# valohai/distributed-llms-example

Hardware: AMD Instinct MI355X
Metric: samples/sec (whole node) T5-base summarization fine-tune at 1/2/4/8 MI355X (higher is better)
Workload: dtype bf16; 1 GPU; model=t5-base, global_batch=512, per_gpu_batch=512, grad_accum=1, seq_len=1024, target_len=128, parallelism=dp1, grad_ckpt=False, grad_dtype=float32, backend=none, world_size=1, comm_stress=False, hip_graph=True

## Files before the change

csrc/attn.hip:

```cpp
#include "common.h"
#include "route.h"
#include "attn_params.h"
#include "attn_tile.h"
#include <stdlib.h>
#include <type_traits>

using namespace dllm;

DLLM_SEED_STEP_TU(attn)

namespace {

static_assert(HG == RW_G, "attention Weyl step = the row-Weyl hash's");
DLLM_DEVICE uint32_t pair_y(uint32_t g) { return rw_pair_y(g); }
DLLM_DEVICE uint32_t pair_gbase(uint32_t rh, uint32_t kp0) { return rw_gbase(rh, kp0); }
DLLM_DEVICE uint32_t drop_mask2(uint32_t y, uint32_t t2) { return rw_drop2(y, t2); }

DLLM_DEVICE constexpr int keep_bit(int t, int i) { return ((i & 1) << 4) + 8 * t + (i >> 1); }
DLLM_DEVICE uint32_t pair_slot_kp(int p) { return (uint32_t)((p & 1) + 4 * ((p & 7) >> 1) + 16 * (p >> 3)); }

DLLM_DEVICE uint32_t dropout_word(uint32_t rh, int kbase, int hh, uint32_t thr) {
  const uint32_t gbase = pair_gbase(rh, (uint32_t)(kbase >> 1) + 2u * (uint32_t)hh);
  const uint32_t t2 = ((thr - 0x8000u) & 0xFFFFu) * 0x10001u;
  uint32_t drop = 0;
// ... 557 lines not shown
    for (int i = 0; i < 2; ++i) {
      const uint32_t qq = (uint32_t)min(qt * K2_QT + drow[i], P.Sq - 1);
      const uint32_t dst = base + (uint32_t)((2 * w + i) * 1024);
      bld16(qbase_p, __umul24(qq, qss2) + dc16[i], __builtin_amdgcn_readfirstlane(dst));
      bld16(dbase_p, __umul24(qq, dss2) + dc16[i], __builtin_amdgcn_readfirstlane(dst + TILE64 * 2));
    }
    glds4(rec_src + (long)qt * 256, __builtin_amdgcn_readfirstlane(base + 4 * TILE64 + w * 256));
    if (DROP) glds4(keep_src + qt * K2_QT, __builtin_amdgcn_readfirstlane(base + 4 * TILE64 + 1024 + w * 256));
  };
  constexpr int DPT = DROP ? 6 : 5;

  if (qt_begin < nqt_all) issue(0, qt_begin);
  if (NB == 3 && qt_begin + 1 < nqt_all) issue(1, qt_begin + 1);
  if (HAS_BIAS) {
    const float* lrow = P.lut + (long)h * L;
    for (int t = tid; t < win + K2_QT; t += 256) {
      const int i = win - 1 - t, gi = k0 + i;
      lut_r[t] = (i >= 0 && gi < L) ? lrow[gi] * LOG2E : 0.f;
    }
    for (int i = tid; i < win; i += 256) dlut_s[i] = 0.f;
  }
  float sat_acc_lo = 0.f, sat_acc_hi = 0.f;
  bool key_ok = false;
  if (tid < BWD_BK) {
    const int kk = k0 + tid;
    key_ok = kk < P.Sk;
    if (HAS_KPM && key_ok) key_ok = P.kpm[(long)b * P.Sk + kk] != 0;
    kmask[tid] = key_ok ? 0.f : -INFINITY;
  }
  const bool block_live = !HAS_KPM || __syncthreads_or(key_ok ? 1 : 0);
  const bool block_masked = __syncthreads_or((tid < BWD_BK && !key_ok) ? 1 : 0);
  bf16x8v kf[4], vf[4];
  {
    const uint16_t* kp = P.k + b * P.k_sb + (long)key * P.k_ss + h * P.k_sh;
    const uint16_t* vp = P.v + b * P.v_sb + (long)key * P.v_ss + h * P.v_sh;
#pragma unroll
    for (int s = 0; s < 4; ++s) {
      u16x8 a = {0, 0, 0, 0, 0, 0, 0, 0}, c = a;
      if (kvalid) {
        a = *reinterpret_cast<const u16x8*>(kp + 16 * s + 8 * hh);
        c = *reinterpret_cast<const u16x8*>(vp + 16 * s + 8 * hh);
      }
      kf[s] = as_frag(a);
      vf[s] = as_frag(c);
    }
  }
  asm volatile("" ::"v"(kf[0]), "v"(kf[1]), "v"(kf[2]), "v"(kf[3]), "v"(vf[0]), "v"(vf[1]), "v"(vf[2]), "v"(vf[3]));
  const float km = kmask[w * 32 + r];
  const int kl = key - k0, kc = kl & 31;
  const int mcol = (kl >> 6) * 2 + ((kc >> 2) & 1);
  const int mbit = keep_bit((kl >> 5) & 1, (kc & 3) + 4 * (kc >> 3));
  const float dscale = DROP ? 1.f / (1.f - P.p_drop) : 1.f;
  const uint32_t dsbits = __float_as_uint(dscale);

  const int nqt = block_live ? nqt_all : qt_begin;
  if (!block_live) wait_vm<0>();
  f32x16 dv0 = {}, dv1 = {}, dk0 = {}, dk1 = {};
  auto stage = [&](int qt, auto slot_c) __attribute__((always_inline)) {
    constexpr int SLOT = decltype(slot_c)::value;
    if (NB == 3 && qt + 1 < nqt) wait_vm<DPT>();
    else wait_vm<0>();
    __syncthreads();
    if (qt + NB - 1 < nqt) issue((SLOT + NB - 1) % NB, qt + NB - 1);
    const unsigned char* stg = smem + SLOT * K2_STAGE;
    const uint16_t* Qb = reinterpret_cast<const uint16_t*>(stg);
    const uint16_t* dOb = Qb + TILE64;
    const float* rec = reinterpret_cast<const float*>(stg + 4 * TILE64);
    const uint32_t* mwd = reinterpret_cast<const uint32_t*>(stg + 4 * TILE64 + 1024);
#pragma unroll
    for (int u = 0; u < 2; ++u) {
      const int q0 = qt * K2_QT + 32 * u;
      f32x16 sacc = {}, dpacc = {};
      if constexpr (NB == 3) {
        bf16x8v qa[4], da[4];
#pragma unroll
        for (int s = 0; s < 4; ++s) {
          qa[s] = as_frag(ld_row(Qb, 32 * u + r, 2 * s + hh));
          da[s] = as_frag(ld_row(dOb, 32 * u + r, 2 * s + hh));
        }
        __builtin_amdgcn_sched_barrier(0);
#pragma unroll
        for (int s = 0; s < 4; ++s) {
          sacc = mfma32(qa[s], kf[s], sacc);
          dpacc = mfma32(da[s], vf[s], dpacc);
        }
      } else {
#pragma unroll
        for (int s = 0; s < 4; ++s) {
          sacc = mfma32(as_frag(ld_row(Qb, 32 * u + r, 2 * s + hh)), kf[s], sacc);
          dpacc = mfma32(as_frag(ld_row(dOb, 32 * u + r, 2 * s + hh)), vf[s], dpacc);
        }
      }
      const int sat = !HAS_BIAS ? 0
                      : (kw0 + 31 - q0 + P.Sq - 1 <= P.sat_lo ? 1 : (kw0 - q0 - 31 + P.Sq - 1 >= P.sat_hi ? 2 : 0));
      const bool use_lut = HAS_BIAS && sat == 0;
      f32x16 pd, ds;
      if constexpr (NB == 3) {
        const float* rt_row = rec + (use_lut ? 0 : (sat == 1 ? 64 : 128)) + 32 * u + 4 * hh;
        const float* nd_row = rec + 192 + 32 * u + 4 * hh;
        float rt[16], nd[16];
        uint32_t mw[16];
#pragma unroll
        for (int g = 0; g < 4; ++g) {
          const f32x4 a = *reinterpret_cast<const f32x4*>(rt_row + 8 * g);
          const f32x4 c = *reinterpret_cast<const f32x4*>(nd_row + 8 * g);
#pragma unroll
          for (int e = 0; e < 4; ++e) {
            rt[4 * g + e] = a[e];
            nd[4 * g + e] = c[e];
          }
          if (DROP) {
            const u32x4 v = *reinterpret_cast<const u32x4*>(mwd + mcol * 64 + 32 * u + 8 * g + 4 * hh);
#pragma unroll
            for (int e = 0; e < 4; ++e) mw[4 * g + e] = v[e];
          }
        }
        if (use_lut) {
          const float* lrow_t = lut_r + (win - 1 - (key - q0 - 4 * hh + P.Sq - 1 - k0));
#pragma unroll
          for (int i0 = 0; i0 < 16; i0 += 8) {
            float lv[8];
#pragma unroll
            for (int i = 0; i < 8; ++i) lv[i] = lrow_t[crow(i0 + i, 0)];
#pragma unroll
            for (int i = 0; i < 8; ++i) rt[i0 + i] += lv[i];
          }
        }
        if (block_masked) {
#pragma unroll
          for (int i = 0; i < 16; ++i) rt[i] += km;
        }
        const bool tile_causal = CAUSAL && (kw0 + 31 > q0 + P.causal_off);
#pragma unroll
        for (int i = 0; i < 16; ++i) {
          const float x = fmaf(sacc[i], sl2, rt[i]);
          float pr = fast_exp2(x);
          if (CAUSAL && tile_causal && key > q0 + crow(i, hh) + P.causal_off) pr = 0.f;
          float keepf = 1.f;
          if (DROP) keepf = __uint_as_float((uint32_t)__builtin_amdgcn_sbfe((int)mw[i], mbit, 1) & dsbits);
          pd[i] = pr * keepf;
          ds[i] = pr * fmaf(dpacc[i], keepf, nd[i]);
        }
      } else {
        const float* rt_row = rec + (use_lut ? 0 : (sat == 1 ? 64 : 128)) + 32 * u + 4 * hh;
        const float* nd_row = rec + 192 + 32 * u + 4 * hh;
        const float* lrow_t = lut_r + (win - 1 - (key - q0 - 4 * hh + P.Sq - 1 - k0));
        const bool tile_causal = CAUSAL && (kw0 + 31 > q0 + P.causal_off);
#pragma unroll
        for (int g = 0; g < 4; ++g) {
          f32x4 rt4 = *reinterpret_cast<const f32x4*>(rt_row + 8 * g);
          const f32x4 nd4 = *reinterpret_cast<const f32x4*>(nd_row + 8 * g);
          u32x4 mw4 = {0u, 0u, 0u, 0u};
          if (DROP) mw4 = *reinterpret_cast<const u32x4*>(mwd + mcol * 64 + 32 * u + 8 * g + 4 * hh);
#pragma unroll
          for (int e = 0; e < 4; ++e) {
            const int i = 4 * g + e;
            float t = rt4[e];
            if (use_lut) t += lrow_t[crow(i, 0)];
            if (block_masked) t += km;
            float pr = fast_exp2(fmaf(sacc[i], sl2, t));
            if (CAUSAL && tile_causal && key > q0 + crow(i, hh) + P.causal_off) pr = 0.f;
            float keepf = 1.f;
            if (DROP) keepf = __uint_as_float((uint32_t)__builtin_amdgcn_sbfe((int)mw4[e], mbit, 1) & dsbits);
            sacc[i] = pr * keepf;
            dpacc[i] = pr * fmaf(dpacc[i], keepf, nd4[e]);
          }
        }
        pd = sacc;
        ds = dpacc;
      }
      if (HAS_BIAS && sat != 0) {
        float t = 0.f;
#pragma unroll
        for (int i = 0; i < 16; ++i) t += ds[i];
        if (sat == 1) sat_acc_lo += t;
        else sat_acc_hi += t;
      } else if (HAS_BIAS) {
        const int rb = r + 4 * hh;
        float tot = 0.f, neg = 0.f;
#pragma unroll
        for (int i0 = 0; i0 < 16; i0 += 8) {
          float v[8];
#pragma unroll
          for (int i = 0; i < 8; ++i) v[i] = __shfl(ds[i0 + i], ((rb + crow(i0 + i, 0)) & 31) + 32 * hh, 64);
#pragma unroll
          for (int i = 0; i < 8; ++i) {
            tot += v[i];
            neg += rb + crow(i0 + i, 0) < 32 ? 0.f : v[i];
          }
        }
        tot += __shfl_xor(tot, 32, 64);
        neg += __shfl_xor(neg, 32, 64);
        const int li = w * 32 + r - q0 + P.Sq - 1;
        const int la = hh == 0 ? li : li - 32;
        const float va = hh == 0 ? tot - neg : (li >= 32 ? neg : 0.f);
        atomicAdd(&dlut_s[la < 0 ? 0 : la], va);
      }
      const bf16x8v pf0 = pack8(pd, 0), pf1 = pack8(pd, 8), sf0 = pack8(ds, 0), sf1 = pack8(ds, 8);
      if constexpr (NB == 3) {
        bf16x8v ot[2][2], qtr[2][2];
#pragma unroll
        for (int sp = 0; sp < 2; ++sp) {
          const int c0 = 32 * u + 16 * sp + 4 * hh;
#pragma unroll
          for (int t = 0; t < 2; ++t) {
            ot[sp][t] = ld_tr_operand(dOb, c0, t, r);
            qtr[sp][t] = ld_tr_operand(Qb, c0, t, r);
          }
        }
        __builtin_amdgcn_sched_barrier(0);
#pragma unroll
        for (int sp = 0; sp < 2; ++sp) {
          const bf16x8v pfv = sp == 0 ? pf0 : pf1, sfv = sp == 0 ? sf0 : sf1;
          dv0 = mfma32(ot[sp][0], pfv, dv0);
          dv1 = mfma32(ot[sp][1], pfv, dv1);
          dk0 = mfma32(qtr[sp][0], sfv, dk0);
          dk1 = mfma32(qtr[sp][1], sfv, dk1);
        }
      } else {
#pragma unroll
        for (int sp = 0; sp < 2; ++sp) {
          const int c0 = 32 * u + 16 * sp + 4 * hh;
          const bf16x8v pfv = sp == 0 ? pf0 : pf1, sfv = sp == 0 ? sf0 : sf1;
          dv0 = mfma32(ld_tr_operand(dOb, c0, 0, r), pfv, dv0);
          dv1 = mfma32(ld_tr_operand(dOb, c0, 1, r), pfv, dv1);
          dk0 = mfma32(ld_tr_operand(Qb, c0, 0, r), sfv, dk0);
          dk1 = mfma32(ld_tr_operand(Qb, c0, 1, r), sfv, dk1);
        }
      }
    }
  };
  for (int qt = qt_begin; qt < nqt; qt += NB) {
    stage(qt, std::integral_constant<int, 0>{});
    if (qt + 1 < nqt) stage(qt + 1, std::integral_constant<int, 1>{});
    if constexpr (NB == 3) {
      if (qt + 2 < nqt) stage(qt + 2, std::integral_constant<int, 2>{});
    }
  }

  {
    __syncthreads();
    unsigned char* scr = smem + w * 8192;
#pragma unroll
    for (int t = 0; t < 2; ++t) {
      const f32x16& ak = t == 0 ? dk0 : dk1;
      const f32x16& av = t == 0 ? dv0 : dv1;
#pragma unroll
      for (int g = 0; g < 4; ++g) {
        u16x4 pk = {f2bf(ak[4 * g] * P.scale), f2bf(ak[4 * g + 1] * P.scale), f2bf(ak[4 * g + 2] * P.scale),
                    f2bf(ak[4 * g + 3] * P.scale)};
        u16x4 pv = {f2bf(av[4 * g]), f2bf(av[4 * g + 1]), f2bf(av[4 * g + 2]), f2bf(av[4 * g + 3])};
        const int off = r * 128 + (((4 * t + g) ^ (r & 7)) << 4) + 8 * hh;
        *reinterpret_cast<u16x4*>(scr + off) = pk;
        *reinterpret_cast<u16x4*>(scr + 4096 + off) = pv;
      }
    }
    asm volatile("s_waitcnt lgkmcnt(0)" ::: "memory");
    float ak[8] = {0.f, 0.f, 0.f, 0.f, 0.f, 0.f, 0.f, 0.f}, av[8] = {0.f, 0.f, 0.f, 0.f, 0.f, 0.f, 0.f, 0.f};
#pragma unroll
    for (int st = 0; st < 4; ++st) {
      const int row = 8 * st + (lane >> 3), ch = lane & 7;
      const int off = row * 128 + ((ch ^ (row & 7)) << 4);
      const u16x8 vk = *reinterpret_cast<const u16x8*>(scr + off);
      const u16x8 vv = *reinterpret_cast<const u16x8*>(scr + 4096 + off);
      const int ks = kw0 + row;
      if (ks < P.Sk) {
        *reinterpret_cast<u16x8*>(P.dk + b * P.dk_sb + (long)ks * P.dk_ss + h * P.dk_sh + 8 * ch) = vk;
        *reinterpret_cast<u16x8*>(P.dv + b * P.dv_sb + (long)ks * P.dv_ss + h * P.dv_sh + 8 * ch) = vv;
        if constexpr (CS) {
          cs_add(ak, vk);
          cs_add(av, vv);
        }
      }
    }
    if constexpr (CS) {
      float* red = reinterpret_cast<float*>(smem + 4 * 8192);
      cs_wave(ak, lane, red + w * 128);
      cs_wave(av, lane, red + w * 128 + 64);
      __syncthreads();
      if (tid < 128) {
        const int c = tid & 63, which = tid >> 6;
        const float s = red[which * 64 + c] + red[128 + which * 64 + c] + red[256 + which * 64 + c] +
                        red[384 + which * 64 + c];
        (which == 0 ? P.csk : P.csv)[(long)(b * P.n_tiles + kblk) * P.cskv_ld + h * 64 + c] = s;
      }
    }
  }
  if (HAS_BIAS) {
    __syncthreads();
    float* grow = P.dlut + (long)h * L;
    for (int i = tid; i < win; i += 256) {
      const int gi = k0 + i;
      const float v = dlut_s[i];
      if (gi < L && v != 0.f) atomicAdd(grow + gi, v);
    }
    const float a_lo = wave_sum(sat_acc_lo), a_hi = wave_sum(sat_acc_hi);
    if (lane == 0) {
      if (a_lo != 0.f) atomicAdd(grow, a_lo);
      if (a_hi != 0.f) atomicAdd(grow + L - 1, a_hi);
    }
  }
}

template <bool HAS_KPM, bool DROP, int MB, bool CS = false>
__global__ __launch_bounds__(256, 2) void attn_bwd_dkdv_sq_kernel(AttnParams P) {
  extern __shared__ __attribute__((aligned(16))) unsigned char smem[];
  const uint32_t* keepb = reinterpret_cast<const uint32_t*>(smem + 2 * K2_STAGE);
  float* kmask = reinterpret_cast<float*>(smem + 2 * K2_STAGE + 4096);

  const int tid = threadIdx.x, w = __builtin_amdgcn_readfirstlane(tid >> 6), lane = tid & 63, r = lane & 31,
            hh = lane >> 5;
  const int ngrp = (P.n_tiles + MB - 1) / MB;
  const int logical = xcd_remap(blockIdx.x, gridDim.x);
  const int grp = logical % ngrp;
  const int bh = logical / ngrp;
  const int h = bh % P.H, b = bh / P.H;
  const int kb_begin = grp * MB;
  const int kb_end = min(kb_begin + MB, P.n_tiles);
  const float sl2 = P.scale * LOG2E;
  const int nqt = (P.Sq + K2_QT - 1) / K2_QT;
  const uint32_t st_lds = lds_addr(smem);

  {
    const uint16_t* qbase_p = P.q + b * P.q_sb + h * P.q_sh;
    const uint16_t* dbase_p = P.dout + b * P.do_sb + h * P.do_sh;
    const uint32_t qss2 = (uint32_t)P.q_ss * 2u, dss2 = (uint32_t)P.do_ss * 2u;
    const float* rec_src = P.rowrec + (long)bh * (P.sq_pad >> 6) * 256 + w * 64 + lane;
    for (int qt = 0; qt < nqt; ++qt) {
      const uint32_t base = st_lds + (uint32_t)(qt * K2_STAGE);
#pragma unroll
      for (int i = 0; i < 2; ++i) {
        const int drow = 8 * (2 * w + i) + (lane >> 3);
        const uint32_t dc16 = (uint32_t)(((lane & 7) ^ swz(drow)) * 16);
        const uint32_t qq = (uint32_t)min(qt * K2_QT + drow, P.Sq - 1);
        const uint32_t dst = base + (uint32_t)((2 * w + i) * 1024);
        bld16(qbase_p, __umul24(qq, qss2) + dc16, __builtin_amdgcn_readfirstlane(dst));
        bld16(dbase_p, __umul24(qq, dss2) + dc16, __builtin_amdgcn_readfirstlane(dst + TILE64 * 2));
      }
      glds4(rec_src + (long)qt * 256, __builtin_amdgcn_readfirstlane(base + 4 * TILE64 + w * 256));
    }
  }
  const int kl = w * 32 + r, kc = kl & 31;
  const int mcol = (kl >> 6) * 2 + ((kc >> 2) & 1);
  const int mbit = keep_bit((kl >> 5) & 1, (kc & 3) + 4 * (kc >> 3));
  const uint32_t dsbits = __float_as_uint(DROP ? 1.f / (1.f - P.p_drop) : 1.f);

  auto issue_keep = [&](int kb, int par) __attribute__((always_inline)) {
    if constexpr (DROP) {
      const int ktf = min(2 * kb + (w >> 1), P.n_ktiles - 1);
      const uint32_t* src = P.dmask + (((long)bh * P.n_ktiles + ktf) * 2 + (w & 1)) * P.sq_pad + lane;
      for (int qt = 0; qt < nqt; ++qt)
        glds4(src + qt * K2_QT,
              __builtin_amdgcn_readfirstlane(st_lds + 2 * K2_STAGE + (uint32_t)((par * 2 + qt) * 1024 + w * 256)));
    }
  };
  auto load_kv = [&](int kb, bf16x8v(&kf)[4], bf16x8v(&vf)[4]) __attribute__((always_inline)) {
    const int key = kb * BWD_BK + kl;
    const bool kvalid = key < P.Sk;
    const uint16_t* kp = P.k + b * P.k_sb + (long)key * P.k_ss + h * P.k_sh;
    const uint16_t* vp = P.v + b * P.v_sb + (long)key * P.v_ss + h * P.v_sh;
#pragma unroll
    for (int s = 0; s < 4; ++s) {
      u16x8 a = {0, 0, 0, 0, 0, 0, 0, 0}, c = a;
      if (kvalid) {
        a = *reinterpret_cast<const u16x8*>(kp + 16 * s + 8 * hh);
        c = *reinterpret_cast<const u16x8*>(vp + 16 * s + 8 * hh);
      }
      kf[s] = as_frag(a);
      vf[s] = as_frag(c);
    }
  };
  auto key_flag = [&](int kb) __attribute__((always_inline)) {
    const int kk = kb * BWD_BK + tid;
    bool ok = tid < BWD_BK && kk < P.Sk;
    if (HAS_KPM && ok) ok = P.kpm[(long)b * P.Sk + kk] != 0;
    return ok;
  };

  bf16x8v kf[4], vf[4], kfn[4], vfn[4];
  issue_keep(kb_begin, 0);
  load_kv(kb_begin, kf, vf);
  bool key_ok = key_flag(kb_begin);
  wait_vm<0>();
  __syncthreads();
  for (int kb = kb_begin; kb < kb_end; ++kb) {
    const int par = (kb - kb_begin) & 1;
    if (tid < BWD_BK) kmask[tid] = key_ok ? 0.f : -INFINITY;
    const bool block_live = !HAS_KPM || __syncthreads_or(key_ok ? 1 : 0);
    const bool block_masked = __syncthreads_or((tid < BWD_BK && !key_ok) ? 1 : 0);
    const float km = block_masked ? kmask[kl] : 0.f;
    const bool more = kb + 1 < kb_end;
    if (more) {
      issue_keep(kb + 1, par ^ 1);
      load_kv(kb + 1, kfn, vfn);
      key_ok = key_flag(kb + 1);
    }
    f32x16 dv0 = {}, dv1 = {}, dk0 = {}, dk1 = {};
    if (block_live) {
      for (int qt = 0; qt < nqt; ++qt) {
        const unsigned char* stg = smem + qt * K2_STAGE;
        const uint16_t* Qb = reinterpret_cast<const uint16_t*>(stg);
        const uint16_t* dOb = Qb + TILE64;
        const float* rec = reinterpret_cast<const float*>(stg + 4 * TILE64);
        const uint32_t* mwd = keepb + (par * 2 + qt) * 256;
#pragma unroll
        for (int u = 0; u < 2; ++u) {
          f32x16 sacc = {}, dpacc = {};
#pragma unroll
          for (int s = 0; s < 4; ++s) {
            sacc = mfma32(as_frag(ld_row(Qb, 32 * u + r, 2 * s + hh)), kf[s], sacc);
            dpacc = mfma32(as_frag(ld_row(dOb, 32 * u + r, 2 * s + hh)), vf[s], dpacc);
          }
          const float* rt_row = rec + 128 + 32 * u + 4 * hh;
          const float* nd_row = rec + 192 + 32 * u + 4 * hh;
#pragma unroll
          for (int g = 0; g < 4; ++g) {
            const f32x4 rt4 = *reinterpret_cast<const f32x4*>(rt_row + 8 * g);
            const f32x4 nd4 = *reinterpret_cast<const f32x4*>(nd_row + 8 * g);
            u32x4 mw4 = {0u, 0u, 0u, 0u};
            if (DROP) mw4 = *reinterpret_cast<const u32x4*>(mwd + mcol * 64 + 32 * u + 8 * g + 4 * hh);
#pragma unroll
            for (int e = 0; e < 4; ++e) {
              const int i = 4 * g + e;
              const float pr = fast_exp2(fmaf(sacc[i], sl2, rt4[e] + km));
              float keepf = 1.f;
              if (DROP) keepf = __uint_as_float((uint32_t)__builtin_amdgcn_sbfe((int)mw4[e], mbit, 1) & dsbits);
              sacc[i] = pr * keepf;
              dpacc[i] = pr * fmaf(dpacc[i], keepf, nd4[e]);
            }
          }
          const bf16x8v pf0 = pack8(sacc, 0), pf1 = pack8(sacc, 8), sf0 = pack8(dpacc, 0), sf1 = pack8(dpacc, 8);
#pragma unroll
          for (int sp = 0; sp < 2; ++sp) {
            const int c0 = 32 * u + 16 * sp + 4 * hh;
            const bf16x8v pfv = sp == 0 ? pf0 : pf1, sfv = sp == 0 ? sf0 : sf1;
            dv0 = mfma32(ld_tr_operand(dOb, c0, 0, r), pfv, dv0);
            dv1 = mfma32(ld_tr_operand(dOb, c0, 1, r), pfv, dv1);
            dk0 = mfma32(ld_tr_operand(Qb, c0, 0, r), sfv, dk0);
            dk1 = mfma32(ld_tr_operand(Qb, c0, 1, r), sfv, dk1);
          }
        }
      }
    }
    wait_vm<0>();
    __syncthreads();
    {
      unsigned char* scr = smem + 2 * K2_STAGE + 4096 + BWD_BK * 4 + w * 8192;
#pragma unroll
      for (int t = 0; t < 2; ++t) {
        const f32x16& ak = t == 0 ? dk0 : dk1;
        const f32x16& av = t == 0 ? dv0 : dv1;
#pragma unroll
        for (int g = 0; g < 4; ++g) {
          u16x4 pk = {f2bf(ak[4 * g] * P.scale), f2bf(ak[4 * g + 1] * P.scale), f2bf(ak[4 * g + 2] * P.scale),
                      f2bf(ak[4 * g + 3] * P.scale)};
          u16x4 pv = {f2bf(av[4 * g]), f2bf(av[4 * g + 1]), f2bf(av[4 * g + 2]), f2bf(av[4 * g + 3])};
          const int off = r * 128 + (((4 * t + g) ^ (r & 7)) << 4) + 8 * hh;
          *reinterpret_cast<u16x4*>(scr + off) = pk;
          *reinterpret_cast<u16x4*>(scr + 4096 + off) = pv;
        }
      }
      asm volatile("s_waitcnt lgkmcnt(0)" ::: "memory");
      float ak[8] = {0.f, 0.f, 0.f, 0.f, 0.f, 0.f, 0.f, 0.f}, av[8] = {0.f, 0.f, 0.f, 0.f, 0.f, 0.f, 0.f, 0.f};
#pragma unroll
      for (int st = 0; st < 4; ++st) {
        const int row = 8 * st + (lane >> 3), ch = lane & 7;
        const int off = row * 128 + ((ch ^ (row & 7)) << 4);
        const u16x8 vk = *reinterpret_cast<const u16x8*>(scr + off);
        const u16x8 vv = *reinterpret_cast<const u16x8*>(scr + 4096 + off);
        const int ks = kb * BWD_BK + w * 32 + row;
        if (ks < P.Sk) {
          *reinterpret_cast<u16x8*>(P.dk + b * P.dk_sb + (long)ks * P.dk_ss + h * P.dk_sh + 8 * ch) = vk;
          *reinterpret_cast<u16x8*>(P.dv + b * P.dv_sb + (long)ks * P.dv_ss + h * P.dv_sh + 8 * ch) = vv;
          if constexpr (CS) {
            cs_add(ak, vk);
            cs_add(av, vv);
          }
        }
      }
      if constexpr (CS) {
        float* red = reinterpret_cast<float*>(smem + 2 * K2_STAGE + 4096 + BWD_BK * 4 + 4 * 8192);
        cs_wave(ak, lane, red + w * 128);
        cs_wave(av, lane, red + w * 128 + 64);
        __syncthreads();
        if (tid < 128) {
          const int c = tid & 63, which = tid >> 6;
          const float s = red[which * 64 + c] + red[128 + which * 64 + c] + red[256 + which * 64 + c] +
                          red[384 + which * 64 + c];
          (which == 0 ? P.csk : P.csv)[(long)(b * P.n_tiles + kb) * P.cskv_ld + h * 64 + c] = s;
        }
      }
    }
    if (more) {
#pragma unroll
      for (int s = 0; s < 4; ++s) {
        kf[s] = kfn[s];
        vf[s] = vfn[s];
      }
    }
  }
}

#define DISPATCH4(FN, hb, hk, ca, dr, ...)                                              \
  do {                                                                                  \
    if (hb) {                                                                           \
      if (hk) { if (ca) { if (dr) FN<true, true, true, true>(__VA_ARGS__); else FN<true, true, true, false>(__VA_ARGS__); } \
                else { if (dr) FN<true, true, false, true>(__VA_ARGS__); else FN<true, true, false, false>(__VA_ARGS__); } } \
      else { if (ca) { if (dr) FN<true, false, true, true>(__VA_ARGS__); else FN<true, false, true, false>(__VA_ARGS__); } \
             else { if (dr) FN<true, false, false, true>(__VA_ARGS__); else FN<true, false, false, false>(__VA_ARGS__); } } \
    } else {                                                                            \
      if (hk) { if (ca) { if (dr) FN<false, true, true, true>(__VA_ARGS__); else FN<false, true, true, false>(__VA_ARGS__); } \
                else { if (dr) FN<false, true, false, true>(__VA_ARGS__); else FN<false, true, false, false>(__VA_ARGS__); } } \
      else { if (ca) { if (dr) FN<false, false, true, true>(__VA_ARGS__); else FN<false, false, true, false>(__VA_ARGS__); } \
             else { if (dr) FN<false, false, false, true>(__VA_ARGS__); else FN<false, false, false, false>(__VA_ARGS__); } } \
    }                                                                                   \
  } while (0)

template <bool HB, bool HK, bool CA, bool DR>
void launch_fwd_t(const AttnParams& p, int nblk, size_t lds, hipStream_t st) {
  const size_t lds2 = lds - (size_t)2 * TILE64 * 2 - FWD_PAD * 4;
  if (3 * lds2 <= 160 * 1024)
    hipLaunchKernelGGL((attn_fwd_kernel<HB, HK, CA, DR, 2>), dim3(nblk), dim3(256), lds2, st, p);
  else
    hipLaunchKernelGGL((attn_fwd_kernel<HB, HK, CA, DR, 3>), dim3(nblk), dim3(256), lds, st, p);
}
template <bool HB, bool HK, bool CA, bool DR>
void launch_bwd_dq_t(const AttnParams& p, int nblk, size_t lds, hipStream_t st) {
  if constexpr (!HB) {
    if (p.csq != nullptr) {
      hipLaunchKernelGGL((attn_bwd_dq_kernel<HB, HK, CA, DR, 2, true>), dim3(nblk), dim3(256), lds, st, p);
      return;
    }
  }
  hipLaunchKernelGGL((attn_bwd_dq_kernel<HB, HK, CA, DR, 2>), dim3(nblk), dim3(256), lds, st, p);
}
template <bool HB, bool HK, bool CA, bool DR>
void launch_bwd_dkdv2_t(const AttnParams& p, int nblk, size_t lds, hipStream_t st) {
  const size_t lds2 = lds - K2_STAGE;
  if (!HB && (!DR || p.Sq <= 256) && 3 * lds2 <= 160 * 1024) {
    if constexpr (!HB) {
      if (p.csk != nullptr) {
        hipLaunchKernelGGL((attn_bwd_dkdv2_kernel<HB, HK, CA, DR, 2, true>), dim3(nblk), dim3(256), lds2, st, p);
        return;
      }
    }
    hipLaunchKernelGGL((attn_bwd_dkdv2_kernel<HB, HK, CA, DR, 2>), dim3(nblk), dim3(256), lds2, st, p);
    return;
  }
  if constexpr (!HB) {
    if (p.csk != nullptr) {
      hipLaunchKernelGGL((attn_bwd_dkdv2_kernel<HB, HK, CA, DR, 3, true>), dim3(nblk), dim3(256), lds, st, p);
      return;
    }
  }
  static size_t attr = 64 * 1024;
  if (lds > attr) {
    (void)hipFuncSetAttribute((const void*)attn_bwd_dkdv2_kernel<HB, HK, CA, DR, 3>,
                              hipFuncAttributeMaxDynamicSharedMemorySize, (int)lds);
    attr = lds;
  }
  hipLaunchKernelGGL((attn_bwd_dkdv2_kernel<HB, HK, CA, DR, 3>), dim3(nblk), dim3(256), lds, st, p);
}

template <bool HK, bool DR, int MB, bool CS>
void launch_bwd_dkdv_sq_cs(const AttnParams& p, dim3 grid, size_t lds, hipStream_t st) {
  static bool attr = false;
  if (!attr) {
    (void)hipFuncSetAttribute((const void*)attn_bwd_dkdv_sq_kernel<HK, DR, MB, CS>,
                              hipFuncAttributeMaxDynamicSharedMemorySize, (int)lds);
    attr = true;
  }
  hipLaunchKernelGGL((attn_bwd_dkdv_sq_kernel<HK, DR, MB, CS>), grid, dim3(256), lds, st, p);
}

template <bool HK, bool DR, int MB>
void launch_bwd_dkdv_sq_mb(const AttnParams& p, dim3 grid, size_t lds, hipStream_t st) {
  if (p.csk != nullptr) launch_bwd_dkdv_sq_cs<HK, DR, MB, true>(p, grid, lds, st);
  else launch_bwd_dkdv_sq_cs<HK, DR, MB, false>(p, grid, lds, st);
}

template <bool HK, bool DR>
void launch_bwd_dkdv_sq_t(const AttnParams& p, int mb, size_t lds, hipStream_t st) {
  const long ng = (p.n_tiles + mb - 1) / mb;
  const dim3 grid((unsigned)(ng * p.H * p.B));
  if (mb >= 8) launch_bwd_dkdv_sq_mb<HK, DR, 8>(p, grid, lds, st);
  else if (mb >= 4) launch_bwd_dkdv_sq_mb<HK, DR, 4>(p, grid, lds, st);
  else launch_bwd_dkdv_sq_mb<HK, DR, 2>(p, grid, lds, st);
}

}

static bool kv_offsets_fit(const AttnParams& p) {
  const long kss2 = p.k_ss * 2, vss2 = p.v_ss * 2;
  return kss2 > 0 && vss2 > 0 && kss2 < (1L << 24) && vss2 < (1L << 24) && p.Sk < (1 << 24) &&
         (long)p.Sk * (kss2 > vss2 ? kss2 : vss2) + 256 < (1L << 31);
}

extern "C" int dllm_attn_fwd(AttnParams* pp, hipStream_t st) {
  AttnParams p = *pp;
  if (!kv_offsets_fit(p)) return -6;
  p.thr = drop_threshold(p.p_drop);
  p.n_tiles = (p.Sq + FWD_BM - 1) / FWD_BM;
  const long nblk = (long)p.n_tiles * p.H * p.B;
  p.n_ktiles = (p.Sk + FWD_BN - 1) / FWD_BN;
  p.sq_pad = p.n_tiles * FWD_BM;
  if (p.p_drop > 0.f && p.dmask == nullptr) return -5;
  size_t lds = (size_t)6 * TILE64 * 2 + 3 * FWD_PAD * 4 + (size_t)p.n_ktiles * (FWD_BN + 1) * 4;
  if (p.lut) lds += (size_t)(p.Sk + FWD_BM + FWD_BN) * 4;
  if (nblk <= 0 || nblk > 0x7fffffff || lds > 160 * 1024) return -4;
  DISPATCH4(launch_fwd_t, p.lut != nullptr, p.kpm != nullptr, p.causal != 0, p.p_drop > 0.f, p, (int)nblk, lds, st);
  DLLM_CHECK_LAUNCH();
  return 0;
}

extern "C" int dllm_attn_bwd(AttnParams* pp, hipStream_t st) {
  AttnParams p = *pp;
  if (!kv_offsets_fit(p)) return -6;
  p.thr = drop_threshold(p.p_drop);
  p.n_tiles = (p.Sq + FWD_BM - 1) / FWD_BM;
  p.n_ktiles = (p.Sk + FWD_BN - 1) / FWD_BN;
  p.sq_pad = p.n_tiles * FWD_BM;
  if (p.p_drop > 0.f && p.dmask == nullptr) return -5;
  if ((p.csq != nullptr || p.csk != nullptr) && (p.rowrec == nullptr || p.lut != nullptr)) return -7;
  if ((p.csk == nullptr) != (p.csv == nullptr)) return -7;
  long nblk = (long)p.n_tiles * p.H * p.B;
  size_t lds = (size_t)4 * TILE64 * 2 + (size_t)p.n_ktiles * (FWD_BN + 1) * 4;
  if (p.lut) lds += (size_t)(p.Sk + FWD_BM + FWD_BN) * 4;
  if (nblk <= 0 || nblk > 0x7fffffff || lds > 160 * 1024) return -4;
  DISPATCH4(launch_bwd_dq_t, p.lut != nullptr, p.kpm != nullptr, p.causal != 0, p.p_drop > 0.f, p, (int)nblk, lds,
            st);
  DLLM_CHECK_LAUNCH();
  p.n_tiles = (p.Sk + BWD_BK - 1) / BWD_BK;
  nblk = (long)p.n_tiles * p.H * p.B;
  constexpr int sq_cap = 4;
  static const int cus = [] {
    int dev = 0, n = 0;
    (void)hipGetDevice(&dev);
    (void)hipDeviceGetAttribute(&n, hipDeviceAttributeMultiprocessorCount, dev);
    return n > 0 ? n : 256;
  }();
  const bool force = route_int("attn_dkdv_sq_force", 0) == 1;
  int mb = 0;
  for (int m = 8; m >= 2; m /= 2)
    if (m <= sq_cap && mb == 0 && (force || (long)((p.n_tiles + m - 1) / m) * p.H * p.B >= 6L * cus)) mb = m;
  if (p.rowrec != nullptr && p.lut == nullptr && !p.causal && p.Sq <= 2 * K2_QT && mb > 1 && p.n_tiles >= 2) {
    const size_t lds_sq = (size_t)2 * K2_STAGE + 4096 + BWD_BK * 4 + 4 * 8192 + 2048;
    if ((long)((p.n_tiles + mb - 1) / mb) * p.H * p.B > 0x7fffffff) return -4;
    if (p.kpm != nullptr) {
      if (p.p_drop > 0.f) launch_bwd_dkdv_sq_t<true, true>(p, mb, lds_sq, st);
      else launch_bwd_dkdv_sq_t<true, false>(p, mb, lds_sq, st);
    } else {
      if (p.p_drop > 0.f) launch_bwd_dkdv_sq_t<false, true>(p, mb, lds_sq, st);
      else launch_bwd_dkdv_sq_t<false, false>(p, mb, lds_sq, st);
    }
    DLLM_CHECK_LAUNCH();
    return 0;
  }
  if (p.rowrec == nullptr) return -5;
  lds = (size_t)K2_NBUF * K2_STAGE + BWD_BK * 4;
  if (p.lut) lds += (size_t)(2 * (p.Sq + BWD_BK) + K2_QT) * 4;
  if (nblk <= 0 || nblk > 0x7fffffff || lds > 160 * 1024) return -4;
  DISPATCH4(launch_bwd_dkdv2_t, p.lut != nullptr, p.kpm != nullptr, p.causal != 0, p.p_drop > 0.f, p, (int)nblk,
            lds, st);
  DLLM_CHECK_LAUNCH();
  return 0;
}

extern "C" int dllm_attn_dropout_mask(AttnParams* pp, hipStream_t st) {
  AttnParams p = *pp;
  if (p.p_drop <= 0.f || p.dmask == nullptr) return -5;
  p.thr = drop_threshold(p.p_drop);
  p.n_ktiles = (p.Sk + FWD_BN - 1) / FWD_BN;
  p.sq_pad = (p.Sq + FWD_BM - 1) / FWD_BM * FWD_BM;
  const long nwords = (long)p.B * p.H * p.n_ktiles * 2 * p.sq_pad;
  const int blocks = (int)std::min<long>((nwords + 255) / 256, 65536);
  hipLaunchKernelGGL(attn_dropout_mask_kernel, dim3(blocks), dim3(256), 0, st, p, nwords);
  DLLM_CHECK_LAUNCH();
  return 0;
}
```

csrc/attn_tile.h:

```cpp
#pragma once
#include "common.h"

typedef __attribute__((ext_vector_type(8))) __bf16 bf16x8v;
typedef __attribute__((ext_vector_type(4))) short s16x4;
typedef __attribute__((ext_vector_type(8))) float f32x8;

namespace {

using namespace dllm;

constexpr int D = 64;
constexpr int TILE64 = 64 * D;
constexpr int TILE32 = 32 * D;
constexpr int FWD_BM = 128;
constexpr int FWD_BN = 64;
constexpr int BWD_BK = 128;
constexpr int BWD_BQ = 32;
constexpr float LOG2E = 1.4426950408889634f;
constexpr float LN2 = 0.6931471805599453f;
constexpr float RESCALE_THR = 8.f;
constexpr uint32_t HG = 0x9E3779B1u;

DLLM_DEVICE bf16x8v as_frag(u16x8 v) { return __builtin_bit_cast(bf16x8v, v); }

DLLM_DEVICE float fast_exp2(float x) { return __builtin_amdgcn_exp2f(x); }

DLLM_DEVICE bf16x8v pack8(const f32x16& a, int base) {
  const f32x8 v = {a[base], a[base + 1], a[base + 2], a[base + 3], a[base + 4], a[base + 5], a[base + 6], a[base + 7]};
  return __builtin_convertvector(v, bf16x8v);
}

DLLM_DEVICE f32x16 mfma32(bf16x8v a, bf16x8v b, f32x16 c) {
  return __builtin_amdgcn_mfma_f32_32x32x16_bf16(a, b, c, 0, 0, 0);
}

DLLM_DEVICE int xcd_remap(int bid, int nblk) {
  const int q = nblk / 8, r = nblk % 8, x = bid % 8;
  return (x < r ? x * (q + 1) : r * (q + 1) + (x - r) * q) + bid / 8;
}

DLLM_DEVICE int crow(int reg, int hh) { return (reg & 3) + 8 * (reg >> 2) + 4 * hh; }

DLLM_DEVICE int swz(int r) { return (((r >> 1) & 1) << 2) | ((r >> 2) & 3); }
DLLM_DEVICE int toff(int r, int c) { return (r << 6) + ((c ^ swz(r)) << 3); }
DLLM_DEVICE u16x8 ld_row(const uint16_t* T, int r, int c) { return *reinterpret_cast<const u16x8*>(T + toff(r, c)); }
DLLM_DEVICE void st_row(uint16_t* T, int r, int c, u16x8 v) { *reinterpret_cast<u16x8*>(T + toff(r, c)) = v; }

DLLM_DEVICE u16x4 ld_tr(const uint16_t* T, int r0, int c0, int i) {
  const int r = r0 + (i >> 2);
  const int col = c0 + 4 * (i & 3);
  const int off = (r << 6) + (((col >> 3) ^ swz(r)) << 3) + (col & 4);
  s16x4 v = __builtin_amdgcn_ds_read_tr16_b64_v4i16((__attribute__((address_space(3))) s16x4*)(T + off));
  return __builtin_bit_cast(u16x4, v);
}

DLLM_DEVICE bf16x8v ld_tr_operand(const uint16_t* T, int kb0, int t, int r) {
  const int c0 = 32 * t + 16 * ((r >> 4) & 1);
  const u16x4 lo = ld_tr(T, kb0, c0, r & 15);
  const u16x4 hi = ld_tr(T, kb0 + 8, c0, r & 15);
  const u16x8 v = {lo.x, lo.y, lo.z, lo.w, hi.x, hi.y, hi.z, hi.w};
  return as_frag(v);
}

}
```

distributed_llms_example_amd/ops/routing.py:

```python
from __future__ import annotations

import os

DEFAULTS: dict = {
    "proj_fwd": "lib",
    "proj_fwd_min_rows": 131072,
    "proj_dgrad": "rows",
    "proj_dgrad_min_rows": 16384,
    "wgrad_min_rows": 4096,
    "ffn": "fused",
    "ffn_min_rows": 1025,
    "ffn_w4_min_rows": 0,
    "ffn_gelu": "pp",
    "gated_min_mf": 2 * 256 * 256 * 256,
    "gated_max_d": 1024,
    "lmhead": "auto",
    "lmhead_full_mb": 16384.0,
    "lmhead_chunk_mb": 128.0,
    "attn_f32": 1,
    "attn_hd": 1,
    "attn_chunk": 0,
    "attn_chunk_min": 8192,
    "wgrad_stream": "auto",
    "wgrad_stream_max_tokens": 32768,
    "wgrad_stream_lag": 2,
    "wgrad_stream_sites": "",
    "gen_fused_beam": 1,
    "gen_shared_cross": 1,
    "gen_check_every": 8,
    "gen_host": 0,
    "reducer": "native",
    "rebuild_buckets": 1,
    "graph_comm": "",
    "eval_batch": 256,
    "gemm_grp": 4,
    "attn_dkdv_sq_force": 0,
    "w4_sched": 769,
}

_cache: tuple[str, dict] | None = None


def overrides() -> dict:
    global _cache
    raw = os.environ.get("DLLM_ROUTE", "")
    if _cache is not None and _cache[0] == raw:
        return _cache[1]
    out = {}
    for item in filter(None, (x.strip() for x in raw.split(","))):
        k, _, v = item.partition("=")
        k = k.strip()
        if k not in DEFAULTS:
            raise KeyError(f"DLLM_ROUTE: unknown key {k!r} (known: {', '.join(sorted(DEFAULTS))})")
        d = DEFAULTS[k]
        out[k] = type(d)(float(v)) if isinstance(d, (int, float)) and not isinstance(d, bool) else v.strip()
    _cache = (raw, out)
    return out


def merged(**kw) -> str:
    cur = dict(overrides())
    for k, v in kw.items():
        if k not in DEFAULTS:
            raise KeyError(f"unknown route key {k!r}")
        cur[k] = v
    return ",".join(f"{k}={v}" for k, v in cur.items())


def get(key: str):
    ov = overrides()
    return ov[key] if key in ov else DEFAULTS[key]


def attention_route(head_dim: int, bf16: bool = True) -> str:
    if head_dim == 64:
        return "attn.hip" if bf16 else ("attn_f32.hip" if get("attn_f32") else "composite")
    if bf16 and 32 <= head_dim <= 128 and head_dim % 8 == 0 and get("attn_hd"):
        return "attn_hd.hip"
    return "composite"


def plan(model: str, tokens_enc: int, tokens_dec: int, d_model: int, d_ff: int, act: str, vocab: int, *,
         head_dim: int = 64) -> dict:
    rows = {"enc": tokens_enc, "dec": tokens_dec}
    out = {}
    dmode = get("proj_dgrad")
    for side, r in rows.items():
        out[f"{side}.wgrad"] = "w4-wgrad" if r >= get("wgrad_min_rows") else "hipblaslt"
        fm = get("proj_fwd")
        out[f"{side}.proj_fwd"] = ("w4" if fm == "w4" else "w4-narrow" if fm == "narrow" and r >= get("proj_fwd_min_rows")
                                   else "hipblaslt")
        if dmode == "w4":
            dg = "w4"
        elif dmode == "lib":
            dg = "hipblaslt"
        else:
            dg = "w4" if r >= get("proj_dgrad_min_rows") else "hipblaslt"
        out[f"{side}.proj_dgrad"] = dg
        if get("ffn") != "fused" or r < get("ffn_min_rows"):
            out[f"{side}.ffn"] = "hipblaslt+act"
        elif act == "relu":
            out[f"{side}.ffn"] = "w4-relu" if r >= get("ffn_w4_min_rows") else "pingpong-relu+w4-drelu"
        elif act in ("gelu", "gelu_new", "gelu_fast") and not act.startswith("gated"):
            out[f"{side}.ffn"] = "w4-gelu" if get("ffn_gelu") == "w4" else "pingpong-gelu"
        else:
            out[f"{side}.ffn"] = ("pingpong-geglu" if r * d_ff >= get("gated_min_mf") and d_model <= get("gated_max_d")
                                  else "hipblaslt+act")
    logits_mb = tokens_dec * vocab * 2 / 2**20
    lm = get("lmhead")
    out["lm_head"] = ("w4-fused-ce" if lm == "fused" or (lm == "auto" and logits_mb > get("lmhead_full_mb"))
                      else "hipblaslt+ce")
    out["attention"] = attention_route(head_dim)
    return out
```

Before: 1027 samples/s.

## Fuse dQ computation into short-query dK/dV backward kernel as one-pass path

Adds a DQ variant of the short-query dK/dV backward kernel. One block per (batch, head) loops over all key blocks, computes delta in-kernel from dO and O, stages K and dS transposed in LDS, and accumulates dQ via extra MFMAs. The separate dQ backward launch is skipped when the shape qualifies (short Sq, enough batch*heads for the CU count). This removes a kernel launch and the recomputation of S/dP in the dQ kernel. In exchange, parallelism drops to one block per head and the inner loop gains extra barriers and serialised K/V loads.

```diff
diff --git a/csrc/attn.hip b/csrc/attn.hip
--- a/csrc/attn.hip
+++ b/csrc/attn.hip
@@ -883,23 +883,27 @@
   }
 }
 
-template <bool HAS_KPM, bool DROP, int MB, bool CS = false>
+template <bool HAS_KPM, bool DROP, int MB, bool CS = false, bool DQ = false, int NQT = 0>
 __global__ __launch_bounds__(256, 2) void attn_bwd_dkdv_sq_kernel(AttnParams P) {
   extern __shared__ __attribute__((aligned(16))) unsigned char smem[];
   const uint32_t* keepb = reinterpret_cast<const uint32_t*>(smem + 2 * K2_STAGE);
   float* kmask = reinterpret_cast<float*>(smem + 2 * K2_STAGE + 4096);
+  unsigned char* stage_scr = smem + 2 * K2_STAGE + 4096 + BWD_BK * 4;
+  uint16_t* Kt = reinterpret_cast<uint16_t*>(stage_scr);
+  uint16_t* dSt = Kt + 2 * TILE64;
 
   const int tid = threadIdx.x, w = __builtin_amdgcn_readfirstlane(tid >> 6), lane = tid & 63, r = lane & 31,
             hh = lane >> 5;
-  const int ngrp = (P.n_tiles + MB - 1) / MB;
+  int ngrp = 1;
+  if constexpr (!DQ) ngrp = (P.n_tiles + MB - 1) / MB;
   const int logical = xcd_remap(blockIdx.x, gridDim.x);
   const int grp = logical % ngrp;
   const int bh = logical / ngrp;
   const int h = bh % P.H, b = bh / P.H;
-  const int kb_begin = grp * MB;
-  const int kb_end = min(kb_begin + MB, P.n_tiles);
+  const int kb_begin = DQ ? 0 : grp * MB;
+  const int kb_end = DQ ? P.n_tiles : min(kb_begin + MB, P.n_tiles);
   const float sl2 = P.scale * LOG2E;
-  const int nqt = (P.Sq + K2_QT - 1) / K2_QT;
+  const int nqt = DQ ? NQT : (P.Sq + K2_QT - 1) / K2_QT;
   const uint32_t st_lds = lds_addr(smem);
 
   {
@@ -918,7 +922,33 @@
         bld16(qbase_p, __umul24(qq, qss2) + dc16, __builtin_amdgcn_readfirstlane(dst));
         bld16(dbase_p, __umul24(qq, dss2) + dc16, __builtin_amdgcn_readfirstlane(dst + TILE64 * 2));
       }
-      glds4(rec_src + (long)qt * 256, __builtin_amdgcn_readfirstlane(base + 4 * TILE64 + w * 256));
+      if constexpr (!DQ)
+        glds4(rec_src + (long)qt * 256, __builtin_amdgcn_readfirstlane(base + 4 * TILE64 + w * 256));
+    }
+  }
+  if constexpr (DQ) {
+    const int row = tid >> 1, hp = tid & 1;
+    const bool qv = row < P.Sq;
+    const uint16_t* dp = P.dout + b * P.do_sb + (long)row * P.do_ss + h * P.do_sh;
+    const uint16_t* op = P.o + b * P.o_sb + (long)row * P.o_ss + h * P.o_sh;
+    float dpart = 0.f;
+#pragma unroll
+    for (int s = 0; s < 4; ++s) {
+      u16x8 c = {0, 0, 0, 0, 0, 0, 0, 0}, o8 = c;
+      if (qv) {
+        c = *reinterpret_cast<const u16x8*>(dp + 16 * s + 8 * hp);
+        o8 = *reinterpret_cast<const u16x8*>(op + 16 * s + 8 * hp);
+      }
+#pragma unroll
+      for (int j = 0; j < 8; ++j) dpart += bf2f(c[j]) * bf2f(o8[j]);
+    }
+    const float delta = dpart + __shfl_xor(dpart, 1, 64);
+    const long row_g = (long)bh * P.Sq + row;
+    const float lse2 = qv ? P.lse[row_g] : INFINITY;
+    if (qv && hp == 0) P.delta[row_g] = delta;
+    if ((row >> 6) < nqt) {
+      float* rec = reinterpret_cast<float*>(smem + (row >> 6) * K2_STAGE + 4 * TILE64);
+      rec[(hp == 0 ? 128 : 192) + (row & 63)] = hp == 0 ? -lse2 : (qv ? -delta : 0.f);
     }
   }
   const int kl = w * 32 + r, kc = kl & 31;
@@ -959,12 +989,23 @@
   };
 
   bf16x8v kf[4], vf[4], kfn[4], vfn[4];
+  f32x16 dqa0 = {}, dqa1 = {};
+  const int trc = 16 * ((r >> 4) & 1);
+  const uint16_t* kt_lo = tr_ptr(Kt, 4 * hh, 32 * (w >> 1) + trc, r & 15);
+  const uint16_t* kt_hi = tr_ptr(Kt, 4 * hh + 8, 32 * (w >> 1) + trc, r & 15);
+  const uint16_t* ds_lo = tr_ptr(dSt, 4 * hh, 32 * (w & 1) + trc, r & 15);
+  const uint16_t* ds_hi = tr_ptr(dSt, 4 * hh + 8, 32 * (w & 1) + trc, r & 15);
   issue_keep(kb_begin, 0);
   load_kv(kb_begin, kf, vf);
   bool key_ok = key_flag(kb_begin);
   wait_vm<0>();
   __syncthreads();
+  const int lane_o = lane, r_o = r, hh_o = hh, kl_o = kl, tid_o = tid;
   for (int kb = kb_begin; kb < kb_end; ++kb) {
+    int lane_v = lane_o;
+    if constexpr (DQ) asm volatile("" : "+v"(lane_v));
+    const int lane = lane_v, r = DQ ? lane_v & 31 : r_o, hh = DQ ? lane_v >> 5 : hh_o, kl = DQ ? w * 32 + r : kl_o;
+    const int tid = DQ ? w * 64 + lane_v : tid_o;
     const int par = (kb - kb_begin) & 1;
     if (tid < BWD_BK) kmask[tid] = key_ok ? 0.f : -INFINITY;
     const bool block_live = !HAS_KPM || __syncthreads_or(key_ok ? 1 : 0);
@@ -973,12 +1014,28 @@
     const bool more = kb + 1 < kb_end;
     if (more) {
       issue_keep(kb + 1, par ^ 1);
-      load_kv(kb + 1, kfn, vfn);
+      if constexpr (!DQ) load_kv(kb + 1, kfn, vfn);
       key_ok = key_flag(kb + 1);
     }
     f32x16 dv0 = {}, dv1 = {}, dk0 = {}, dk1 = {};
-    if (block_live) {
-      for (int qt = 0; qt < nqt; ++qt) {
+    if constexpr (DQ) {
+      if (block_live) {
+#pragma unroll
+        for (int s = 0; s < 4; ++s) st_row(Kt, kl, 2 * s + hh, __builtin_bit_cast(u16x8, kf[s]));
+      }
+    }
+    auto load_kv_next = [&](int kbn) __attribute__((always_inline)) {
+      const int key = min(kbn * BWD_BK + kl, P.Sk - 1);
+      const uint16_t* kp = P.k + b * P.k_sb + (long)key * P.k_ss + h * P.k_sh;
+      const uint16_t* vp = P.v + b * P.v_sb + (long)key * P.v_ss + h * P.v_sh;
+#pragma unroll
+      for (int s = 0; s < 4; ++s) {
+        kf[s] = as_frag(*reinterpret_cast<const u16x8*>(kp + 16 * s + 8 * hh));
+        vf[s] = as_frag(*reinterpret_cast<const u16x8*>(vp + 16 * s + 8 * hh));
+      }
+    };
+    auto stage = [&](auto qt_c, auto last_c, f32x16& dqa) __attribute__((always_inline)) {
+        const int qt = qt_c;
         const unsigned char* stg = smem + qt * K2_STAGE;
         const uint16_t* Qb = reinterpret_cast<const uint16_t*>(stg);
         const uint16_t* dOb = Qb + TILE64;
@@ -989,8 +1046,8 @@
           f32x16 sacc = {}, dpacc = {};
 #pragma unroll
           for (int s = 0; s < 4; ++s) {
-            sacc = mfma32(as_frag(ld_row(Qb, 32 * u + r, 2 * s + hh)), kf[s], sacc);
-            dpacc = mfma32(as_frag(ld_row(dOb, 32 * u + r, 2 * s + hh)), vf[s], dpacc);
+            sacc = mfma32(as_frag(ld_row(Qb + u * TILE32, r, 2 * s + hh)), kf[s], sacc);
+            dpacc = mfma32(as_frag(ld_row(dOb + u * TILE32, r, 2 * s + hh)), vf[s], dpacc);
           }
           const float* rt_row = rec + 128 + 32 * u + 4 * hh;
           const float* nd_row = rec + 192 + 32 * u + 4 * hh;
@@ -1011,22 +1068,52 @@
             }
           }
           const bf16x8v pf0 = pack8(sacc, 0), pf1 = pack8(sacc, 8), sf0 = pack8(dpacc, 0), sf1 = pack8(dpacc, 8);
+          if constexpr (DQ) {
+            if (u == 0 && qt > 0) __syncthreads();
+            const u16x8 s0v = __builtin_bit_cast(u16x8, sf0), s1v = __builtin_bit_cast(u16x8, sf1);
+            uint16_t* drow = dSt + (kl << 6) + 4 * hh;
+            const int sw = swz(kl);
+            *reinterpret_cast<u16x4*>(drow + (((4 * u + 0) ^ sw) << 3)) = u16x4{s0v[0], s0v[1], s0v[2], s0v[3]};
+            *reinterpret_cast<u16x4*>(drow + (((4 * u + 1) ^ sw) << 3)) = u16x4{s0v[4], s0v[5], s0v[6], s0v[7]};
+            *reinterpret_cast<u16x4*>(drow + (((4 * u + 2) ^ sw) << 3)) = u16x4{s1v[0], s1v[1], s1v[2], s1v[3]};
+            *reinterpret_cast<u16x4*>(drow + (((4 * u + 3) ^ sw) << 3)) = u16x4{s1v[4], s1v[5], s1v[6], s1v[7]};
+          }
 #pragma unroll
           for (int sp = 0; sp < 2; ++sp) {
-            const int c0 = 32 * u + 16 * sp + 4 * hh;
+            const int c0 = (32 * u + 16 * sp) * D;
             const bf16x8v pfv = sp == 0 ? pf0 : pf1, sfv = sp == 0 ? sf0 : sf1;
-            dv0 = mfma32(ld_tr_operand(dOb, c0, 0, r), pfv, dv0);
-            dv1 = mfma32(ld_tr_operand(dOb, c0, 1, r), pfv, dv1);
-            dk0 = mfma32(ld_tr_operand(Qb, c0, 0, r), sfv, dk0);
-            dk1 = mfma32(ld_tr_operand(Qb, c0, 1, r), sfv, dk1);
+            dv0 = mfma32(ld_tr_operand(dOb + c0, 4 * hh, 0, r), pfv, dv0);
+            dv1 = mfma32(ld_tr_operand(dOb + c0, 4 * hh, 1, r), pfv, dv1);
+            dk0 = mfma32(ld_tr_operand(Qb + c0, 4 * hh, 0, r), sfv, dk0);
+            dk1 = mfma32(ld_tr_operand(Qb + c0, 4 * hh, 1, r), sfv, dk1);
           }
         }
-      }
+        if constexpr (DQ) {
+          if (decltype(last_c)::value) {
+            __builtin_amdgcn_sched_barrier(0);
+            if (more) load_kv_next(kb + 1);
+          }
+          __syncthreads();
+#pragma unroll
+          for (int j = 0; j < 8; ++j)
+            dqa = mfma32(ld_tr_pair(kt_lo + j * 1024, kt_hi + j * 1024), ld_tr_pair(ds_lo + j * 1024, ds_hi + j * 1024),
+                         dqa);
+        }
+    };
+    if (block_live) {
+      if constexpr (DQ) {
+        stage(std::integral_constant<int, 0>{}, std::integral_constant<bool, NQT == 1>{}, dqa0);
+        if constexpr (NQT > 1) stage(std::integral_constant<int, 1>{}, std::true_type{}, dqa1);
+      } else {
+        for (int qt = 0; qt < nqt; ++qt) stage(qt, std::false_type{}, dqa0);
+      }
+    } else if constexpr (DQ) {
+      if (more) load_kv_next(kb + 1);
     }
     wait_vm<0>();
     __syncthreads();
     {
-      unsigned char* scr = smem + 2 * K2_STAGE + 4096 + BWD_BK * 4 + w * 8192;
+      unsigned char* scr = stage_scr + w * 8192;
 #pragma unroll
       for (int t = 0; t < 2; ++t) {
         const f32x16& ak = t == 0 ? dk0 : dk1;
@@ -1060,7 +1147,7 @@
         }
       }
       if constexpr (CS) {
-        float* red = reinterpret_cast<float*>(smem + 2 * K2_STAGE + 4096 + BWD_BK * 4 + 4 * 8192);
+        float* red = reinterpret_cast<float*>(stage_scr + 4 * 8192);
         cs_wave(ak, lane, red + w * 128);
         cs_wave(av, lane, red + w * 128 + 64);
         __syncthreads();
@@ -1072,11 +1159,46 @@
         }
       }
     }
-    if (more) {
-#pragma unroll
-      for (int s = 0; s < 4; ++s) {
-        kf[s] = kfn[s];
-        vf[s] = vfn[s];
+    if constexpr (!DQ) {
+      if (more) {
+#pragma unroll
+        for (int s = 0; s < 4; ++s) {
+          kf[s] = kfn[s];
+          vf[s] = vfn[s];
+        }
+      }
+    }
+  }
+  if constexpr (DQ) {
+    int lane_v = lane_o;
+    asm volatile("" : "+v"(lane_v));
+    const int lane = lane_v, r = lane_v & 31, hh = lane_v >> 5;
+    float* X = reinterpret_cast<float*>(stage_scr);
+#pragma unroll
+    for (int i = 0; i < 16; ++i) {
+      X[w * 2048 + i * 64 + lane] = dqa0[i];
+      X[w * 2048 + 1024 + i * 64 + lane] = dqa1[i];
+    }
+    __syncthreads();
+    f32x16 a0, a1;
+#pragma unroll
+    for (int i = 0; i < 16; ++i) {
+      a0[i] = X[(w & 1) * 2048 + (w >> 1) * 1024 + i * 64 + lane];
+      a1[i] = X[(2 + (w & 1)) * 2048 + (w >> 1) * 1024 + i * 64 + lane];
+    }
+    __syncthreads();
+    float* red = nullptr;
+    if constexpr (CS) {
+      if (P.csq != nullptr) red = reinterpret_cast<float*>(stage_scr + 4 * 8192);
+    }
+    store_rows_staged(stage_scr + w * 4096, a0, a1, P.scale, r, hh, lane,
+                      P.dq + b * P.dq_sb + (long)(32 * w) * P.dq_ss + h * P.dq_sh, P.dq_ss, P.Sq - 32 * w,
+                      red != nullptr ? red + w * 64 : nullptr);
+    if constexpr (CS) {
+      if (red != nullptr) {
+        __syncthreads();
+        if (tid < 64)
+          P.csq[(long)b * P.csq_ld + h * 64 + tid] = red[tid] + red[64 + tid] + red[128 + tid] + red[192 + tid];
       }
     }
   }
@@ -1143,15 +1265,21 @@
   hipLaunchKernelGGL((attn_bwd_dkdv2_kernel<HB, HK, CA, DR, 3>), dim3(nblk), dim3(256), lds, st, p);
 }
 
-template <bool HK, bool DR, int MB, bool CS>
+template <bool HK, bool DR, int MB, bool CS, bool DQ = false, int NQT = 0>
 void launch_bwd_dkdv_sq_cs(const AttnParams& p, dim3 grid, size_t lds, hipStream_t st) {
   static bool attr = false;
   if (!attr) {
-    (void)hipFuncSetAttribute((const void*)attn_bwd_dkdv_sq_kernel<HK, DR, MB, CS>,
+    (void)hipFuncSetAttribute((const void*)attn_bwd_dkdv_sq_kernel<HK, DR, MB, CS, DQ, NQT>,
                               hipFuncAttributeMaxDynamicSharedMemorySize, (int)lds);
     attr = true;
   }
-  hipLaunchKernelGGL((attn_bwd_dkdv_sq_kernel<HK, DR, MB, CS>), grid, dim3(256), lds, st, p);
+  hipLaunchKernelGGL((attn_bwd_dkdv_sq_kernel<HK, DR, MB, CS, DQ, NQT>), grid, dim3(256), lds, st, p);
+}
+
+template <bool HK, bool DR, bool CS>
+void launch_bwd_dkdv_sq_dq(const AttnParams& p, dim3 grid, size_t lds, hipStream_t st) {
+  if (p.Sq > K2_QT) launch_bwd_dkdv_sq_cs<HK, DR, 0, CS, true, 2>(p, grid, lds, st);
+  else launch_bwd_dkdv_sq_cs<HK, DR, 0, CS, true, 1>(p, grid, lds, st);
 }
 
 template <bool HK, bool DR, int MB>
@@ -1162,6 +1290,12 @@
 
 template <bool HK, bool DR>
 void launch_bwd_dkdv_sq_t(const AttnParams& p, int mb, size_t lds, hipStream_t st) {
+  if (mb == 0) {
+    const dim3 grid((unsigned)((long)p.H * p.B));
+    if (p.csk != nullptr) launch_bwd_dkdv_sq_dq<HK, DR, true>(p, grid, lds, st);
+    else launch_bwd_dkdv_sq_dq<HK, DR, false>(p, grid, lds, st);
+    return;
+  }
   const long ng = (p.n_tiles + mb - 1) / mb;
   const dim3 grid((unsigned)(ng * p.H * p.B));
   if (mb >= 8) launch_bwd_dkdv_sq_mb<HK, DR, 8>(p, grid, lds, st);
@@ -1198,21 +1332,12 @@
   AttnParams p = *pp;
   if (!kv_offsets_fit(p)) return -6;
   p.thr = drop_threshold(p.p_drop);
-  p.n_tiles = (p.Sq + FWD_BM - 1) / FWD_BM;
+  const int n_qtiles = (p.Sq + FWD_BM - 1) / FWD_BM, n_kblocks = (p.Sk + BWD_BK - 1) / BWD_BK;
   p.n_ktiles = (p.Sk + FWD_BN - 1) / FWD_BN;
-  p.sq_pad = p.n_tiles * FWD_BM;
+  p.sq_pad = n_qtiles * FWD_BM;
   if (p.p_drop > 0.f && p.dmask == nullptr) return -5;
   if ((p.csq != nullptr || p.csk != nullptr) && (p.rowrec == nullptr || p.lut != nullptr)) return -7;
   if ((p.csk == nullptr) != (p.csv == nullptr)) return -7;
-  long nblk = (long)p.n_tiles * p.H * p.B;
-  size_t lds = (size_t)4 * TILE64 * 2 + (size_t)p.n_ktiles * (FWD_BN + 1) * 4;
-  if (p.lut) lds += (size_t)(p.Sk + FWD_BM + FWD_BN) * 4;
-  if (nblk <= 0 || nblk > 0x7fffffff || lds > 160 * 1024) return -4;
-  DISPATCH4(launch_bwd_dq_t, p.lut != nullptr, p.kpm != nullptr, p.causal != 0, p.p_drop > 0.f, p, (int)nblk, lds,
-            st);
-  DLLM_CHECK_LAUNCH();
-  p.n_tiles = (p.Sk + BWD_BK - 1) / BWD_BK;
-  nblk = (long)p.n_tiles * p.H * p.B;
   constexpr int sq_cap = 4;
   static const int cus = [] {
     int dev = 0, n = 0;
@@ -1221,12 +1346,28 @@
     return n > 0 ? n : 256;
   }();
   const bool force = route_int("attn_dkdv_sq_force", 0) == 1;
+  const bool sq_shape = p.rowrec != nullptr && p.lut == nullptr && !p.causal && p.Sq <= 2 * K2_QT && n_kblocks >= 2;
+  const bool onepass = sq_shape && route_int("attn_sq_onepass", 1) != 0 && (force || (long)p.H * p.B >= 6L * cus) &&
+                       (p.csq == nullptr) == (p.csk == nullptr);
   int mb = 0;
   for (int m = 8; m >= 2; m /= 2)
-    if (m <= sq_cap && mb == 0 && (force || (long)((p.n_tiles + m - 1) / m) * p.H * p.B >= 6L * cus)) mb = m;
-  if (p.rowrec != nullptr && p.lut == nullptr && !p.causal && p.Sq <= 2 * K2_QT && mb > 1 && p.n_tiles >= 2) {
+    if (m <= sq_cap && mb == 0 && (force || (long)((n_kblocks + m - 1) / m) * p.H * p.B >= 6L * cus)) mb = m;
+  p.n_tiles = n_qtiles;
+  long nblk = (long)p.n_tiles * p.H * p.B;
+  size_t lds = (size_t)4 * TILE64 * 2 + (size_t)p.n_ktiles * (FWD_BN + 1) * 4;
+  if (p.lut) lds += (size_t)(p.Sk + FWD_BM + FWD_BN) * 4;
+  if (nblk <= 0 || nblk > 0x7fffffff || lds > 160 * 1024) return -4;
+  if (!onepass) {
+    DISPATCH4(launch_bwd_dq_t, p.lut != nullptr, p.kpm != nullptr, p.causal != 0, p.p_drop > 0.f, p, (int)nblk, lds,
+              st);
+    DLLM_CHECK_LAUNCH();
+  }
+  p.n_tiles = n_kblocks;
+  nblk = (long)p.n_tiles * p.H * p.B;
+  if (onepass || (sq_shape && mb > 1)) {
+    if (onepass) mb = 0;
     const size_t lds_sq = (size_t)2 * K2_STAGE + 4096 + BWD_BK * 4 + 4 * 8192 + 2048;
-    if ((long)((p.n_tiles + mb - 1) / mb) * p.H * p.B > 0x7fffffff) return -4;
+    if (nblk > 0x7fffffff) return -4;
     if (p.kpm != nullptr) {
       if (p.p_drop > 0.f) launch_bwd_dkdv_sq_t<true, true>(p, mb, lds_sq, st);
       else launch_bwd_dkdv_sq_t<true, false>(p, mb, lds_sq, st);
diff --git a/csrc/attn_tile.h b/csrc/attn_tile.h
--- a/csrc/attn_tile.h
+++ b/csrc/attn_tile.h
@@ -3,6 +3,7 @@
 
 typedef __attribute__((ext_vector_type(8))) __bf16 bf16x8v;
 typedef __attribute__((ext_vector_type(4))) short s16x4;
+typedef __attribute__((ext_vector_type(8))) short s16x8;
 typedef __attribute__((ext_vector_type(8))) float f32x8;
 
 namespace {
@@ -54,6 +55,18 @@
   return __builtin_bit_cast(u16x4, v);
 }
 
+DLLM_DEVICE const uint16_t* tr_ptr(const uint16_t* T, int r0, int c0, int i) {
+  const int r = r0 + (i >> 2);
+  const int col = c0 + 4 * (i & 3);
+  return T + (r << 6) + (((col >> 3) ^ swz(r)) << 3) + (col & 4);
+}
+DLLM_DEVICE bf16x8v ld_tr_pair(const uint16_t* lo, const uint16_t* hi) {
+  const s16x4 a = __builtin_amdgcn_ds_read_tr16_b64_v4i16((__attribute__((address_space(3))) s16x4*)lo);
+  const s16x4 b = __builtin_amdgcn_ds_read_tr16_b64_v4i16((__attribute__((address_space(3))) s16x4*)hi);
+  const s16x8 v = __builtin_shufflevector(a, b, 0, 1, 2, 3, 4, 5, 6, 7);
+  return __builtin_bit_cast(bf16x8v, v);
+}
+
 DLLM_DEVICE bf16x8v ld_tr_operand(const uint16_t* T, int kb0, int t, int r) {
   const int c0 = 32 * t + 16 * ((r >> 4) & 1);
   const u16x4 lo = ld_tr(T, kb0, c0, r & 15);
diff --git a/distributed_llms_example_amd/ops/routing.py b/distributed_llms_example_amd/ops/routing.py
--- a/distributed_llms_example_amd/ops/routing.py
+++ b/distributed_llms_example_amd/ops/routing.py
@@ -35,6 +35,7 @@
     "eval_batch": 256,
     "gemm_grp": 4,
     "attn_dkdv_sq_force": 0,
+    "attn_sq_onepass": 1,
     "w4_sched": 769,
 }
 
```

New measurement: 1038 samples/s (median of 6 runs). 1.1% higher.
